# bmezaris/RetargetVid

Measured on AMD Instinct MI355X. Metric: frames/sec end-to-end saliency+crop on 640x360, higher is better.
Workload: dtype f32

## Files before the change

### retargetvid_amd/csrc/svc_tail.hip

```cpp
#include <math.h>

#include <algorithm>
#include <atomic>
#include <chrono>

#include "hdb_tree.h"
#include "svc_cvlinear.h"
#include "svc_internal.h"

#ifndef TB
#define TB 1024
#endif
#define NW16 (TB / 64)
static_assert(TB % 64 == 0 && (NW16 & (NW16 - 1)) == 0 && NW16 >= 4 && NW16 <= 16,
              "the tail kernels need 4, 8 or 16 wavefronts per workgroup");
#define RING_R 20
#define RING_R1 4
#define DEPTH_SLOT 4096
#define REACH_INF 0x1FFFFu

struct FrameWS {
    uint32_t hdr;
    uint32_t pts;
    uint32_t core;
    uint32_t mst;
    uint32_t ea, eb;
    uint32_t labels;
    uint32_t reach;
    uint32_t srt;
    uint32_t sp, ssz, absc, absw, sdn, evc, evs, dparent;
    uint32_t cup, ctp, cleft, cright, cbirthw, cminw, csize, cdn, csplit, cspa, cspb, cacc, csel, crep, cweight;
    uint32_t total;
};

static FrameWS make_layout(int cap, int mc) {
    FrameWS L;
    uint32_t o = 0;
    auto take = [&](size_t bytes) { uint32_t r = o; o += (uint32_t)((bytes + 63) / 64 * 64); return r; };
    L.hdr = take(128);
    L.pts = take(4u * cap); L.core = take(4u * cap);
    L.mst = take(8u * cap); L.ea = take(8u * cap); L.eb = take(8u * cap);
    L.labels = take(4u * cap); L.reach = take(4u * cap); L.srt = take(16u * cap + 128);
    L.sp = take(2u * cap); L.ssz = take(2u * cap); L.absc = take(2u * cap); L.absw = take(4u * cap);
    L.sdn = take(4u * cap); L.evc = take(2u * cap); L.evs = take(2u * cap);
    L.dparent = take(8u * cap);
    L.cup = take(2u * mc); L.ctp = take(4u * mc); L.cleft = take(4u * mc); L.cright = take(4u * mc);
    L.cbirthw = take(4u * mc); L.cminw = take(4u * mc); L.csize = take(4u * mc);
    L.cdn = take(4u * mc); L.csplit = take(4u * mc); L.cspa = take(4u * mc); L.cspb = take(4u * mc);
    L.cacc = take(8u * mc); L.csel = take(1u * mc);
    L.crep = take(4u * mc); L.cweight = take(4u * mc);
    L.total = o;
    return L;
}

struct TailArgs {
    uint8_t *maps;
    uint8_t *ws;
    size_t ws_stride;
    int slot0;
    const uint16_t *order;
    int n, h, w;
    FDiv dW;
    int mcs, min_samples, select_sum, op_close, clust_filt;
    int prim_pt;
    const uint32_t *ring;
    const int32_t *ring_delta;
    int n_ring, n_ring1;
    const uint16_t *ring_cnt;
    int prim_lvl;
    double *xy;
    int32_t *stats;
    FrameWS L;
};

__device__ __forceinline__ unsigned long long wave_min_u64(unsigned long long v) {
#pragma unroll
    for (int o = 32; o > 0; o >>= 1) {
        unsigned long long t = __shfl_xor(v, o);
        v = t < v ? t : v;
    }
    return v;
}
template <int CTRL, int ROW_MASK>
__device__ __forceinline__ uint32_t dpp_add_u32(uint32_t v) {
    return v + (uint32_t)__builtin_amdgcn_update_dpp(0, (int)v, CTRL, ROW_MASK, 0xF, false);
}
__device__ __forceinline__ uint32_t wave_incl_scan_u32(uint32_t v) {
    v = dpp_add_u32<0x111, 0xF>(v);
    v = dpp_add_u32<0x112, 0xF>(v);
    v = dpp_add_u32<0x114, 0xF>(v);
    v = dpp_add_u32<0x118, 0xF>(v);
    v = dpp_add_u32<0x142, 0xA>(v);
    v = dpp_add_u32<0x143, 0xC>(v);
    return v;
}

__device__ __forceinline__ int wave_sum_i32(int v) {
    return __builtin_amdgcn_readlane((int)wave_incl_scan_u32((uint32_t)v), 63);
}

template <typename T>
__device__ __forceinline__ T *carve(uint8_t *&p, size_t count) {
    T *r = (T *)p;
    p += (count * sizeof(T) + 15) / 16 * 16;
    return r;
}

__device__ __forceinline__ int block_excl_scan(int v, int *lds16, int *tot) {
    const int lane = threadIdx.x & 63, wave = threadIdx.x >> 6;
    const int inc = (int)wave_incl_scan_u32((uint32_t)v);
    if (lane == 63) lds16[wave] = inc;
    __syncthreads();
    int base = 0, total = 0;
#pragma unroll
    for (int i = 0; i < NW16; ++i) {
        int c = lds16[i];
        if (i < wave) base += c;
        total += c;
    }
    __syncthreads();
    *tot = total;
    return base + inc - v;
}

__global__ __launch_bounds__(256) void k_threshold(uint8_t *maps, size_t n, int t) {
    size_t i16 = ((size_t)blockIdx.x * 256 + threadIdx.x) * 16;
    if (i16 >= n) return;
    if (i16 + 16 <= n && (((uintptr_t)(maps + i16)) & 15) == 0) {
        uint4 v = *(uint4 *)(maps + i16);
        uint32_t *p = (uint32_t *)&v;
#pragma unroll
        for (int j = 0; j < 4; ++j) {
            uint32_t x = p[j], r = 0;
#pragma unroll
            for (int b = 0; b < 4; ++b) {
                uint32_t c = (x >> (8 * b)) & 255u;
                r |= ((int)c < t ? 0u : c) << (8 * b);
            }
            p[j] = r;
        }
        *(uint4 *)(maps + i16) = v;
    } else {
        for (size_t i = i16; i < n && i < i16 + 16; ++i) maps[i] = maps[i] < t ? 0 : maps[i];
    }
}

__global__ __launch_bounds__(256) void k_blend(uint8_t *maps, const uint16_t *order, int hw) {
    const int f = order[blockIdx.y];
    uint8_t *cur = maps + (size_t)f * hw;
    const uint8_t *prev = cur - hw;
    for (int i = blockIdx.x * 256 + threadIdx.x; i < hw; i += gridDim.x * 256)
        cur[i] = (uint8_t)(((cur[i] + prev[i]) & 255) >> 1);
}

__global__ __launch_bounds__(256) void k_iou(const int4 *__restrict__ a, const int4 *__restrict__ b, size_t n,
                                             double *__restrict__ out) {
    size_t i = (size_t)blockIdx.x * 256 + threadIdx.x;
    if (i >= n) return;
    int4 A = a[i], B = b[i];
    long long xa = max(A.x, B.x), ya = max(A.y, B.y), xb = min(A.z, B.z), yb = min(A.w, B.w);
    long long inter = max(0LL, xb - xa + 1) * max(0LL, yb - ya + 1);
    long long aa = (long long)(A.z - A.x + 1) * (A.w - A.y + 1), ab = (long long)(B.z - B.x + 1) * (B.w - B.y + 1);
    out[i] = (double)inter / (double)(aa + ab - inter);
}

__global__ __launch_bounds__(256) void k_map_resize(const uint8_t *__restrict__ in, uint8_t *__restrict__ out,
                                                    const int *__restrict__ tab, const uint16_t *__restrict__ order,
                                                    int h, int w, int oh, int ow) {
    const int f = order[blockIdx.y];
    const CvLinear T(tab, oh, ow);
    const uint8_t *src = in + (size_t)f * h * w;
    uint8_t *dst = out + (size_t)f * oh * ow;
    for (int i = blockIdx.x * 256 + threadIdx.x; i < oh * ow; i += gridDim.x * 256) {
        const int oy = i / ow, ox = i - oy * ow;
        int y0, y1, b0, b1, sx, sx1, a0, a1;
        bool inner;
        T.row(oy, h, y0, y1, b0, b1);
        T.col(ox, w, sx, sx1, a0, a1, inner);
        const uint8_t *r0 = src + (size_t)y0 * w, *r1 = src + (size_t)y1 * w;
        dst[i] = CvLinear::blend(r0[sx], r0[sx1], r1[sx], r1[sx1], a0, a1, b0, b1, inner);
    }
}

__global__ __launch_bounds__(256) void k_centre_nearest(const uint8_t *__restrict__ maps, int h, int w, int sh, int sw,
                                                        int factor, double *__restrict__ xy) {
    const int f = blockIdx.x;
    const uint8_t *m = maps + (size_t)f * h * w;
    __shared__ unsigned long long red[3 * 4];
    unsigned long long cnt = 0, sr = 0, sc = 0;
    for (int i = threadIdx.x; i < sh * sw; i += 256) {
        const int r = i / sw, c = i - r * sw;
        if (m[(size_t)min(r * factor, h - 1) * w + min(c * factor, w - 1)]) { ++cnt; sr += r; sc += c; }
    }
#pragma unroll
    for (int o = 32; o > 0; o >>= 1) { cnt += __shfl_xor(cnt, o); sr += __shfl_xor(sr, o); sc += __shfl_xor(sc, o); }
    if ((threadIdx.x & 63) == 0) { red[threadIdx.x >> 6] = cnt; red[4 + (threadIdx.x >> 6)] = sr; red[8 + (threadIdx.x >> 6)] = sc; }
    __syncthreads();
    if (threadIdx.x == 0) {
        cnt = red[0] + red[1] + red[2] + red[3];
        sr = red[4] + red[5] + red[6] + red[7];
        sc = red[8] + red[9] + red[10] + red[11];
        if (cnt) {
            xy[2 * f] = (double)sc / (double)cnt * (double)factor;
            xy[2 * f + 1] = (double)sr / (double)cnt * (double)factor;
        } else {
            xy[2 * f] = xy[2 * f + 1] = __longlong_as_double(0x7FF8000000000000LL);
        }
    }
}

__global__ __launch_bounds__(256) void k_centre_argmax(const uint8_t *__restrict__ maps, int h, int w, FDiv dW, double *__restrict__ xy) {
    const int f = blockIdx.x, hw = h * w;
    const uint8_t *m = maps + (size_t)f * hw;
    __shared__ uint32_t red[4];
    uint32_t best = 0;
    for (int i = threadIdx.x; i < hw; i += 256) best = max(best, ((uint32_t)m[i] << 16) | (uint32_t)(65535 - i));
#pragma unroll
    for (int o = 32; o > 0; o >>= 1) best = max(best, (uint32_t)__shfl_xor((int)best, o));
    if ((threadIdx.x & 63) == 0) red[threadIdx.x >> 6] = best;
    __syncthreads();
    if (threadIdx.x == 0) {
        best = max(max(red[0], red[1]), max(red[2], red[3]));
        if (best >> 16) {
            uint32_t c;
            const uint32_t r = fdivmod(65535u - (best & 0xFFFFu), dW, c);
            xy[2 * f] = (double)c;
            xy[2 * f + 1] = (double)r;
        } else {
            xy[2 * f] = xy[2 * f + 1] = __longlong_as_double(0x7FF8000000000000LL);
        }
    }
}

__device__ __forceinline__ void copy_bytes(uint8_t *__restrict__ dst, const uint8_t *__restrict__ src, int n) {
    if ((((uintptr_t)src | (uintptr_t)dst) & 7) == 0) {
        const int n8 = n >> 3;
        for (int i0 = threadIdx.x; i0 < n8; i0 += 8 * TB) {
            uint2 v[8];
#pragma unroll
            for (int u = 0; u < 8; ++u) {
                const int i = i0 + u * TB;
                v[u] = i < n8 ? ((const uint2 *)src)[i] : make_uint2(0u, 0u);
            }
#pragma unroll
            for (int u = 0; u < 8; ++u) {
                const int i = i0 + u * TB;
                if (i < n8) ((uint2 *)dst)[i] = v[u];
            }
        }
        for (int i = (n8 << 3) + threadIdx.x; i < n; i += TB) dst[i] = src[i];
    } else {
        for (int i = threadIdx.x; i < n; i += TB) dst[i] = src[i];
    }
}

__device__ __forceinline__ void compact_body(const TailArgs &A) {
    const int f = A.order[blockIdx.x];
    __shared__ int lds16[NW16];
    extern __shared__ uint8_t sm_compact[];
    const int hw = A.h * A.w;
    const uint8_t *gmap = A.maps + (size_t)f * hw;
    uint8_t *ws = A.ws + (size_t)(A.slot0 + (int)blockIdx.x) * A.ws_stride;
    uint32_t *pts = (uint32_t *)(ws + A.L.pts);
    int32_t *hdr = (int32_t *)(ws + A.L.hdr);
    uint8_t *map = sm_compact;
    copy_bytes(map, gmap, hw);
    __syncthreads();
    const int per = (hw + TB - 1) / TB;
    const int lo = min(hw, (int)threadIdx.x * per), hi = min(hw, lo + per);
    int cnt = 0;
    for (int i = lo; i < hi; ++i) cnt += map[i] != 0;
    int total;
    int pos = block_excl_scan(cnt, lds16, &total);
    if (cnt) {
        uint32_t c; uint32_t r = fdivmod((uint32_t)lo, A.dW, c);
        for (int i = lo; i < hi; ++i) {
            const uint32_t v = map[i];
            if (v) pts[pos++] = r | (c << 8) | (v << 16);
            if (++c == (uint32_t)A.w) { c = 0; ++r; }
        }
    }
    if (threadIdx.x == 0) {
        hdr[0] = total;
        hdr[1] = 0;
        hdr[2] = -1;
        hdr[3] = (A.clust_filt && total > A.mcs + 1) ? 1 : 0;
        hdr[23] = 0;
        hdr[30] = 0;
    }
}
__global__ __launch_bounds__(TB) void k_compact(TailArgs A) { compact_body(A); }

template <int NI>
__device__ __forceinline__ uint32_t core_kth_regs(const uint16_t *rcl, int N, int r, int c, int k, uint32_t lo, uint32_t hi) {
    const int lane = threadIdx.x & 63;
    uint32_t d[NI];
#pragma unroll
    for (int i = 0; i < NI; ++i) {
        const int j = lane + 64 * i;
        d[i] = 0xFFFFFFFFu;
        if (j < N) {
            const uint32_t u = rcl[j];
            const int dr = (int)(u & 255) - r, dc = (int)(u >> 8) - c;
            d[i] = (uint32_t)(dr * dr + dc * dc);
        }
    }
    auto enough = [&](uint32_t t) -> bool {
        int cnt = 0;
#pragma unroll
        for (int i = 0; i < NI; ++i) cnt += d[i] <= t;
        return wave_sum_i32(cnt) >= k + 1;
    };
    for (uint32_t t = 2 * lo; t < hi; t *= 2) {
        if (enough(t)) { hi = t; break; }
        lo = t + 1;
    }
    while (lo < hi) {
        const uint32_t mid = (lo + hi) >> 1;
        if (enough(mid)) hi = mid; else lo = mid + 1;
    }
    return lo;
}

__device__ __forceinline__ void core_body(const TailArgs &A) {
    const int f = A.order[blockIdx.x];
    uint8_t *ws = A.ws + (size_t)(A.slot0 + (int)blockIdx.x) * A.ws_stride;
    const int32_t *hdr = (const int32_t *)(ws + A.L.hdr);
    if (!hdr[3]) return;
    const int N = hdr[0];
    extern __shared__ uint8_t sm_core[];
    const int hw = A.h * A.w;
    uint8_t *occ = sm_core;
    uint32_t *ring = (uint32_t *)(sm_core + (hw + 15) / 16 * 16);
    int32_t *dl1 = (int32_t *)(ring + A.n_ring);
    __shared__ int n_fb, n_fb2;
    const uint8_t *map = A.maps + (size_t)f * hw;
    const long long tc0 = wall_clock64();
    copy_bytes(occ, map, hw);
    for (int i = threadIdx.x; i < A.n_ring; i += TB) ring[i] = A.ring[i];
    for (int i = threadIdx.x; i < A.n_ring1; i += TB) dl1[i] = A.ring_delta[i];
    if (threadIdx.x == 0) { n_fb = 0; n_fb2 = 0; }
    __syncthreads();
    const uint32_t *pts = (const uint32_t *)(ws + A.L.pts);
    uint32_t *core = (uint32_t *)(ws + A.L.core);
    int32_t *fb = (int32_t *)(ws + A.L.labels);
    int32_t *fb2 = (int32_t *)(ws + A.L.reach);
    int k = A.min_samples > 0 ? A.min_samples : A.mcs;
    k = min(N - 1, k);
    if (k == 0) k = 1;
    const int h = A.h, w = A.w;
    const int nr1 = A.n_ring1;
    for (int pbase = 0; pbase < N; pbase += TB) {
        const int p = pbase + threadIdx.x;
        const bool live = p < N;
        const uint32_t v = live ? pts[p] : 0u;
        const int r = v & 255, c = (v >> 8) & 255;
        const bool interior = r >= RING_R1 && r < h - RING_R1 && c >= RING_R1 && c < w - RING_R1;
        const uint8_t *op = occ + r * w + c;
        int cnt = 0;
        uint32_t res = live ? 0xFFFFFFFFu : 0u;
        for (int i0 = 0; i0 < nr1 && __ballot(res == 0xFFFFFFFFu) != 0ull; i0 += 8) {
            bool hit[8];
            if (interior) {
#pragma unroll
                for (int j = 0; j < 8; ++j) hit[j] = (i0 + j < nr1) && op[dl1[min(i0 + j, nr1 - 1)]] != 0;
            } else {
#pragma unroll
                for (int j = 0; j < 8; ++j) {
                    const uint32_t o = ring[min(i0 + j, nr1 - 1)];
                    const int rr = r + (int)(o & 255) - 128, cc = c + (int)((o >> 8) & 255) - 128;
                    const bool in = (i0 + j < nr1) && (unsigned)rr < (unsigned)h && (unsigned)cc < (unsigned)w;
                    hit[j] = in && occ[in ? rr * w + cc : 0] != 0;
                }
            }
            int add = 0;
#pragma unroll
            for (int j = 0; j < 8; ++j) add += hit[j] ? 1 : 0;
            if (res != 0xFFFFFFFFu) continue;
// ... 1341 lines not shown
                const double tj = readlane_f64(term, j);
                for (uint32_t k = 0; k < sj; ++k) acc += tj;
            }
        }
    }
    if (cur != hdb::NONE16 && lane == 0) t.cacc[cur] = acc;
}

template <bool LDS>
__device__ __forceinline__ int cluster_phase(const TailArgs &A, uint8_t *ws, uint8_t *sm, TreeShared &S, int32_t *hdr,
                                             int N, long long t0) {
    const int tid = threadIdx.x, nthr = blockDim.x;
    const int hw = A.h * A.w;
    hdb::Edge *ea = (hdb::Edge *)(ws + A.L.ea);
    const hdb::Edge *edges = ea;
    hdb::Tree t;
    t.dparent = (uint32_t *)(ws + A.L.dparent);
    t.nclusters = 0; t.n = N;
    if (LDS) {
        uint8_t *p = sm;
        hdb::Edge *el = carve<hdb::Edge>(p, TREE_LDS_CAP);
        t.absw = carve<uint32_t>(p, TREE_LDS_CAP); t.sdn = carve<uint32_t>(p, TREE_LDS_CAP);
        t.sp = carve<uint16_t>(p, TREE_LDS_CAP); t.ssz = carve<uint16_t>(p, TREE_LDS_CAP);
        t.absc = carve<uint16_t>(p, TREE_LDS_CAP); t.evc = carve<uint16_t>(p, TREE_LDS_CAP);
        t.evs = carve<uint16_t>(p, TREE_LDS_CAP);
        t.cacc = carve<double>(p, TREE_LDS_CLUSTERS);
        t.ctp = carve<int32_t>(p, TREE_LDS_CLUSTERS); t.cleft = carve<int32_t>(p, TREE_LDS_CLUSTERS);
        t.cright = carve<int32_t>(p, TREE_LDS_CLUSTERS); t.cbirthw = carve<uint32_t>(p, TREE_LDS_CLUSTERS);
        t.cminw = carve<uint32_t>(p, TREE_LDS_CLUSTERS); t.csize = carve<uint32_t>(p, TREE_LDS_CLUSTERS);
        t.cdn = carve<uint32_t>(p, TREE_LDS_CLUSTERS); t.csplit = carve<uint32_t>(p, TREE_LDS_CLUSTERS);
        t.cspa = carve<uint32_t>(p, TREE_LDS_CLUSTERS); t.cspb = carve<uint32_t>(p, TREE_LDS_CLUSTERS);
        t.crep = carve<int32_t>(p, TREE_LDS_CLUSTERS); t.cup = carve<uint16_t>(p, TREE_LDS_CLUSTERS);
        t.csel = carve<uint8_t>(p, TREE_LDS_CLUSTERS);
        t.cap_clusters = TREE_LDS_CLUSTERS;
        for (int i = tid; i < N - 1; i += nthr) el[i] = ea[i];
        edges = el;
    } else {
        t.sp = (uint16_t *)(ws + A.L.sp); t.ssz = (uint16_t *)(ws + A.L.ssz); t.absc = (uint16_t *)(ws + A.L.absc);
        t.absw = (uint32_t *)(ws + A.L.absw); t.sdn = (uint32_t *)(ws + A.L.sdn);
        t.evc = (uint16_t *)(ws + A.L.evc); t.evs = (uint16_t *)(ws + A.L.evs);
        t.cup = (uint16_t *)(ws + A.L.cup); t.ctp = (int32_t *)(ws + A.L.ctp); t.cleft = (int32_t *)(ws + A.L.cleft);
        t.cright = (int32_t *)(ws + A.L.cright); t.cbirthw = (uint32_t *)(ws + A.L.cbirthw);
        t.cminw = (uint32_t *)(ws + A.L.cminw); t.csize = (uint32_t *)(ws + A.L.csize);
        t.cdn = (uint32_t *)(ws + A.L.cdn); t.csplit = (uint32_t *)(ws + A.L.csplit);
        t.cspa = (uint32_t *)(ws + A.L.cspa); t.cspb = (uint32_t *)(ws + A.L.cspb); t.cacc = (double *)(ws + A.L.cacc);
        t.csel = (uint8_t *)(ws + A.L.csel); t.crep = (int32_t *)(ws + A.L.crep);
        t.cap_clusters = hdb::max_clusters(hw, A.mcs);
    }
    {
        const int per = (N + nthr - 1) / nthr;
        hdb::init_points(t, min(N, tid * per), min(N, tid * per + per));
    }
    __syncthreads();
    const bool built = build_wave(t, edges, N, A.mcs);
    if (tid == 0) hdr[13] = (int)(wall_clock64() - t0);
    if (built) accumulate_wave(t, edges);
    if (tid == 0) {
        const bool ok = built;
        if (ok) S.nsel = hdb::choose(t);
        S.ok = ok;
        hdr[4] = t.nclusters;
        hdr[9] = (int)(wall_clock64() - t0);
    }
    __syncthreads();
    if (!S.ok) return -2;
    t.nclusters = hdr[4];
    const int nsel = S.nsel;
    uint32_t *cweight = (uint32_t *)(ws + A.L.cweight);
    for (int c = tid; c < t.nclusters; c += nthr) cweight[c] = 0;
    __syncthreads();
    const uint32_t *pts = (const uint32_t *)(ws + A.L.pts);
    int32_t *labels = (int32_t *)(ws + A.L.labels);
    for (int p = tid; p < N; p += nthr) {
        const int c = hdb::point_cluster(t, (uint32_t)p, nsel);
        labels[p] = c;
        if (c >= 0) {
            const uint32_t val = pts[p] >> 16;
            if (A.select_sum == 1) atomicAdd(&cweight[c], val); else atomicMax(&cweight[c], val);
        }
    }
    __threadfence_block();
    __syncthreads();
    if (tid == 0) {
        int b = -1;
        for (int c = 0; c < t.nclusters; ++c) {
            if (t.crep[c] != c) continue;
            if (b < 0 || cweight[c] > cweight[b] || (cweight[c] == cweight[b] && hdb::cluster_before(t, c, b))) b = c;
        }
        S.best = b;
        hdr[1] = nsel;
        hdr[2] = b;
        hdr[10] = (int)(wall_clock64() - t0);
    }
    __syncthreads();
    return S.best;
}

#ifndef SORT_LDS_BYTES
#define SORT_LDS_BYTES (104 * 1024)
#endif
#define SORT_NONE 0xFFFFu
#define SORT_SMALL 15

struct SortArrays {
    uint32_t *key, *scan;
    uint16_t *idx, *seg, *lpos, *rpos;
};
struct SortSegs {
    uint16_t *lo[2], *hi[2], *pi, *ls, *rs;
// ... 149 lines not shown
    }
    for (int i = tid; i < n; i += TB) {
        const int lo = a.lpos[i], hi = a.rpos[i];
        const uint32_t k = a.key[i];
        int rank = 0;
        for (int j = lo; j <= hi; ++j) {
            const uint32_t kj = a.key[j];
            rank += (kj < k || (kj == k && j < i)) ? 1 : 0;
        }
        out[lo + rank] = a.idx[i];
    }
    __syncthreads();
}

__device__ __forceinline__ void sort_carve(uint8_t *lds, uint8_t *glob, int n, SortArrays &a, SortSegs &st, int *&sh) {
    uint8_t *p = lds;
    sh = carve<int>(p, NW16 + 4);
    const int nseg = n / 17 + 2;
    for (int g = 0; g < 2; ++g) { st.lo[g] = carve<uint16_t>(p, nseg); st.hi[g] = carve<uint16_t>(p, nseg); st.dep[g] = carve<int16_t>(p, nseg); }
    st.pi = carve<uint16_t>(p, nseg); st.ls = carve<uint16_t>(p, nseg); st.rs = carve<uint16_t>(p, nseg);
    st.vp = carve<uint32_t>(p, nseg); st.K = carve<uint32_t>(p, nseg);
    uint8_t *q = ((size_t)(p - lds) + (size_t)n * 16 + 6 * 16 <= SORT_LDS_BYTES) ? p : glob;
    a.key = carve<uint32_t>(q, n); a.scan = carve<uint32_t>(q, n);
    a.idx = carve<uint16_t>(q, n); a.seg = carve<uint16_t>(q, n); a.lpos = carve<uint16_t>(q, n); a.rpos = carve<uint16_t>(q, n);
}

__device__ __forceinline__ void sort_body(const TailArgs &A) {
    uint8_t *ws = A.ws + (size_t)(A.slot0 + (int)blockIdx.x) * A.ws_stride;
    int32_t *hdr = (int32_t *)(ws + A.L.hdr);
    if (!hdr[3]) return;
    const int n = hdr[0] - 1;
    extern __shared__ uint8_t sm_sort[];
    const long long t0 = wall_clock64();
    const hdb::Edge *mst = (const hdb::Edge *)(ws + A.L.mst);
    hdb::Edge *ea = (hdb::Edge *)(ws + A.L.ea);
    SortArrays a; SortSegs st; int *sh;
    sort_carve(sm_sort, ws + A.L.srt, n, a, st, sh);
    for (int i = threadIdx.x; i < n; i += TB) a.key[i] = mst[i].w;
    uint16_t *perm = (uint16_t *)(ws + A.L.eb);
    np_argsort_block(a, st, n, perm, sh);
    for (int i = threadIdx.x; i < n; i += TB) ea[i] = mst[perm[i]];
    if (threadIdx.x == 0) hdr[8] = (int)(wall_clock64() - t0);
}
__global__ __launch_bounds__(TB) void k_sort(TailArgs A) { sort_body(A); }

__global__ __launch_bounds__(TB) void k_argsort_test(const uint32_t *keys, int n, uint16_t *out, uint8_t *scratch) {
    extern __shared__ uint8_t sm_sort[];
    SortArrays a; SortSegs st; int *sh;
    sort_carve(sm_sort, scratch, n, a, st, sh);
    for (int i = threadIdx.x; i < n; i += TB) a.key[i] = keys[i];
    np_argsort_block(a, st, n, out, sh);
}

__global__ __launch_bounds__(64) void k_tree(TailArgs A) {
    uint8_t *ws = A.ws + (size_t)(A.slot0 + (int)blockIdx.x) * A.ws_stride;
    int32_t *hdr = (int32_t *)(ws + A.L.hdr);
    if (!hdr[3] || hdr[23]) return;
    const int N = hdr[0];
    extern __shared__ uint8_t sm_tree[];
    __shared__ TreeShared S;
    const long long t0 = wall_clock64();
    const long long c0 = clock64();
    int best = -2;
    if (N <= TREE_LDS_CAP) best = cluster_phase<true>(A, ws, sm_tree, S, hdr, N, t0);
    if (best == -2) best = cluster_phase<false>(A, ws, sm_tree, S, hdr, N, t0);
    if (threadIdx.x == 0) { hdr[14] = (int)(clock64() - c0); hdr[15] = (int)(wall_clock64() - t0); }
}

#ifndef TP_CAP
#define TP_CAP 4352
#endif
#ifndef TP_CAP_BIG
#define TP_CAP_BIG 8192
#endif
#define TP_CAP_HUGE 65025
#define TP_NONE 0xFFFFu
enum { TP_SMALL = 0, TP_BIRTH = 1, TP_SPLIT = 2, TP_ABS_A = 3, TP_ABS_B = 4 };

struct TpCl {
    double *acc;
    uint32_t *birthw, *minw, *weight;
    uint16_t *tp, *left, *right, *spa, *spb, *node, *topk, *off, *len;
    int16_t *rep;
    uint8_t *sel;
};

static size_t tp_lds_bytes(int hw, int mcs, int *cap_clusters, int *cap_clusters_huge = nullptr) {
    const int cap = std::min(hw, TP_CAP), capb = std::min(hw, TP_CAP_BIG);
    auto up = [](size_t b) { return (b + 15) / 16 * 16; };
    const size_t small = up((size_t)cap * 2) * 8 + up((size_t)(cap + 256) * 2) + up((size_t)cap * 4) * 3 + up((size_t)((cap + 256) / 16 + 16) * 2) + 64;
    const size_t big = hw > TP_CAP ? up((size_t)capb * 2) * 6 + up((size_t)(capb + 256) * 2) + up((size_t)((capb + 256) / 16 + 16) * 2) + 64 : 0;
    const size_t huge = hw > TP_CAP_BIG ? up((size_t)((hw + 256) / 16 + 16) * 2) + up(((size_t)hw / 256 + 32) * 2) + up(32 * 2) + 64 : 0;
    const size_t per_edge = std::max({small, big, huge});
    int cc = hdb::max_clusters(std::min(hw, TP_CAP_HUGE), mcs);
#ifndef TP_LDS_BUDGET
#define TP_LDS_BUDGET (160 * 1024 - 4096)
#endif
    const size_t budget = TP_LDS_BUDGET;
#ifdef TP_CC_EXACT
    if (per_edge + (size_t)cc * 48 + 512 > budget) cc = std::max(8, (int)((budget > per_edge + 512 ? budget - per_edge - 512 : 0) / 48));
#else
    while (cc > 8 && per_edge + (size_t)cc * 48 + 512 > budget) cc /= 2;
#endif
    *cap_clusters = cc;
    const size_t total = per_edge + (size_t)cc * 48 + 512;
    if (cap_clusters_huge) {
        const size_t room = total > huge + 512 ? (total - huge - 512) / 48 : 0;
        *cap_clusters_huge = (int)std::min<size_t>(room, (size_t)hdb::max_clusters(std::min(hw, TP_CAP_HUGE), mcs));
    }
    return total;
}

__device__ __forceinline__ uint32_t tp_gt_mask16(const uint16_t *p, uint32_t r) {
    const uint4 a = ((const uint4 *)p)[0], b = ((const uint4 *)p)[1];
    const uint32_t v[8] = {a.x, a.y, a.z, a.w, b.x, b.y, b.z, b.w};
    uint32_t m = 0;
#pragma unroll
    for (int i = 0; i < 8; ++i) m |= ((v[i] & 0xFFFFu) > r ? 1u << (2 * i) : 0u) | ((v[i] >> 16) > r ? 2u << (2 * i) : 0u);
    return m;
}
// ... 304 lines not shown
            const uint32_t val = pts[pid] >> 16;
            if (A.select_sum == 1) atomicAdd(&C.weight[lab], val); else atomicMax(&C.weight[lab], val);
        }
    }
    __syncthreads();
    if (tid == 0) {
        auto depth = [&](uint32_t k) { int d = 0; while (par[k] != TP_NONE) { k = par[k]; ++d; } return d; };
        auto before = [&](int c1, int c2) -> bool {
            const uint32_t p1 = C.tp[c1], p2 = C.tp[c2];
            if (p1 == TP_NONE) return true;
            if (p2 == TP_NONE) return false;
            if (p1 == p2) return C.left[p1] == c1;
            uint32_t s1 = C.node[p1], s2 = C.node[p2];
            const int d1 = depth(s1), d2 = depth(s2);
            if (d1 != d2) return d1 < d2;
            uint32_t side1 = 0, side2 = 0;
            while (s1 != s2) {
                side1 = s1 > par[s1]; side2 = s2 > par[s2];
                s1 = par[s1]; s2 = par[s2];
            }
            return side1 < side2;
        };
        int b = -1;
        for (int c = 0; c < nc; ++c) {
            if (C.rep[c] != c) continue;
            if (b < 0 || C.weight[c] > C.weight[b] || (C.weight[c] == C.weight[b] && before(c, b))) b = c;
        }
        hdr[1] = nsel;
        hdr[2] = b;
        hdr[23] = 1;
        hdr[10] = (int)(wall_clock64() - t0);
        hdr[15] = hdr[10];
    }
}
#undef TP_ORDER
#undef TP_W

__device__ __forceinline__ void tree_par_body(const TailArgs &A, int cap_clusters, int cap_clusters_huge) {
    uint8_t *ws = A.ws + (size_t)(A.slot0 + (int)blockIdx.x) * A.ws_stride;
    int32_t *hdr = (int32_t *)(ws + A.L.hdr);
    if (!hdr[3]) return;
    const int N = hdr[0];
    if (N > TP_CAP_HUGE) return;
    extern __shared__ uint8_t sm_tp[];
    __shared__ int lds16[NW16];
    __shared__ int sh_nc, sh_nsel;
    if (N <= TP_CAP) tp_body<0>(A, cap_clusters, ws, hdr, N, sm_tp, lds16, sh_nc, sh_nsel);
    else if (N <= TP_CAP_BIG) tp_body<1>(A, cap_clusters, ws, hdr, N, sm_tp, lds16, sh_nc, sh_nsel);
    else tp_body<2>(A, cap_clusters_huge, ws, hdr, N, sm_tp, lds16, sh_nc, sh_nsel);
}
__global__ __launch_bounds__(TB) void k_tree_par(TailArgs A, int cap_clusters, int cap_clusters_huge) { tree_par_body(A, cap_clusters, cap_clusters_huge); }

__device__ __forceinline__ void finish_body(const TailArgs &A) {
    const int f = A.order[blockIdx.x];
    uint8_t *ws = A.ws + (size_t)(A.slot0 + (int)blockIdx.x) * A.ws_stride;
    int32_t *hdr = (int32_t *)(ws + A.L.hdr);
    if (hdr[30]) return;
    const int N = hdr[0];
    const int hw = A.h * A.w;
    uint8_t *map = A.maps + (size_t)f * hw;
    extern __shared__ uint8_t sm_fin[];
    __shared__ unsigned long long red[3 * NW16];
    __shared__ uint32_t box[4];
    const int tid = threadIdx.x;
    if (tid < 4) box[tid] = 255u;
    const bool clustered = hdr[3] != 0;
    long long t0 = 0;
    if (tid == 0) t0 = wall_clock64();
    const int best = clustered ? hdr[2] : -1;
    uint8_t *m0 = sm_fin;
    uint8_t *m1 = sm_fin + (hw + 15) / 16 * 16;
    copy_bytes(m0, map, hw);
    __syncthreads();
    int wr0 = 0, wc0 = 0, wh = A.h, ww = A.w;
    if (best >= 0) {
        const uint32_t *pts = (const uint32_t *)(ws + A.L.pts);
        const int32_t *labels = (const int32_t *)(ws + A.L.labels);
        uint32_t rmin = 255, cmin = 255, rmaxc = 255, cmaxc = 255;
        for (int p = tid; p < N; p += TB) {
            const uint32_t v = pts[p], r = v & 255, c = (v >> 8) & 255;
            if (labels[p] != best) m0[r * A.w + c] = 0;
            else { rmin = min(rmin, r); cmin = min(cmin, c); rmaxc = min(rmaxc, 255u - r); cmaxc = min(cmaxc, 255u - c); }
        }
        const uint32_t a = wave_min_u32(rmin), b = wave_min_u32(cmin), c_ = wave_min_u32(rmaxc), d = wave_min_u32(cmaxc);
        if ((tid & 63) == 0) { atomicMin(&box[0], a); atomicMin(&box[1], b); atomicMin(&box[2], c_); atomicMin(&box[3], d); }
        __syncthreads();
        if (box[0] <= 255u - box[2]) {
            wr0 = max(0, (int)box[0] - 4); wc0 = max(0, (int)box[1] - 4);
            wh = min(A.h, (int)(255u - box[2]) + 5) - wr0; ww = min(A.w, (int)(255u - box[3]) + 5) - wc0;
        }
        if (A.op_close) {
            close_pass<true, true>(m0, m1, A.w, wr0, wc0, wh, ww);
            __syncthreads();
            close_pass<true, false>(m1, m0, A.w, wr0, wc0, wh, ww);
            __syncthreads();
            close_pass<false, true>(m0, m1, A.w, wr0, wc0, wh, ww);
            __syncthreads();
            close_pass<false, false>(m1, m0, A.w, wr0, wc0, wh, ww);
            __syncthreads();
        }
        copy_bytes(map, m0, hw);
    }
    __syncthreads();
    unsigned long long cnt = 0, sr = 0, sc = 0;
    for (int i = tid; i < wh * ww; i += TB) {
        const int r = wr0 + i / ww, c = wc0 + i % ww;
        if (m0[r * A.w + c]) { ++cnt; sr += (uint32_t)r; sc += (uint32_t)c; }
    }
    cnt = (unsigned long long)(uint32_t)wave_sum_i32((int)cnt);
    sr = (unsigned long long)(uint32_t)wave_sum_i32((int)sr);
    sc = (unsigned long long)(uint32_t)wave_sum_i32((int)sc);
    if ((tid & 63) == 0) { red[tid >> 6] = cnt; red[NW16 + (tid >> 6)] = sr; red[2 * NW16 + (tid >> 6)] = sc; }
    __syncthreads();
    if (tid == 0) {
        cnt = sr = sc = 0;
        for (int i = 0; i < NW16; ++i) { cnt += red[i]; sr += red[NW16 + i]; sc += red[2 * NW16 + i]; }
        if (cnt) {
            A.xy[2 * f] = (double)sc / (double)cnt;
            A.xy[2 * f + 1] = (double)sr / (double)cnt;
        } else {
            A.xy[2 * f] = A.xy[2 * f + 1] = __longlong_as_double(0x7FF8000000000000LL);
        }
        if (A.stats) {
            A.stats[4 * f] = N;
            A.stats[4 * f + 1] = clustered ? hdr[1] : 0;
            A.stats[4 * f + 2] = clustered ? hdr[2] : -1;
            A.stats[4 * f + 3] = (int)cnt;
        }
        hdr[11] = (int)(wall_clock64() - t0);
    }
}
__global__ __launch_bounds__(TB) void k_finish(TailArgs A) { finish_body(A); }

__global__ __launch_bounds__(TB) void k_tail_front(TailArgs A) {
    compact_body(A);
    __syncthreads();
    core_body(A);
    __syncthreads();
    prim_lvl_body(A);
}

__global__ __launch_bounds__(TB) void k_tail_back(TailArgs A, int cap_clusters, int cap_clusters_huge) {
    int32_t *hdr = (int32_t *)(A.ws + (size_t)(A.slot0 + (int)blockIdx.x) * A.ws_stride + A.L.hdr);
    sort_body(A);
    __syncthreads();
    tree_par_body(A, cap_clusters, cap_clusters_huge);
    __syncthreads();
    if (hdr[3] && !hdr[23]) return;
    finish_body(A);
    __syncthreads();
    if (threadIdx.x == 0) hdr[30] = 1;
}

extern "C" int svc_threshold_u8(SvcHandle *h, uint8_t *maps, size_t n_bytes, int t, void *stream) {
    if (!h || (n_bytes > 0 && !maps)) { svc_set_error("svc_threshold_u8: invalid argument"); return SVC_E_INVALID; }
    if (n_bytes == 0) return SVC_OK;
    SVC_HIP(hipSetDevice(h->device));
    ProfScope ps(h, SVC_K_THRESHOLD, (hipStream_t)stream);
    k_threshold<<<(unsigned)((n_bytes + 4095) / 4096), 256, 0, (hipStream_t)stream>>>(maps, n_bytes, t);
    SVC_CHECK_LAUNCH();
    return SVC_OK;
}

extern "C" int svc_iou_i32(const int32_t *a, const int32_t *b, size_t n, double *out, void *stream) {
    if (!a || !b || !out) { svc_set_error("svc_iou_i32: invalid argument"); return SVC_E_INVALID; }
    if (n == 0) return SVC_OK;
    k_iou<<<(unsigned)((n + 255) / 256), 256, 0, (hipStream_t)stream>>>((const int4 *)a, (const int4 *)b, n, out);
    SVC_CHECK_LAUNCH();
    return SVC_OK;
}

static int upload_map_tab(DevBuf &buf, int h, int w, int oh, int ow, double sy, double sx) {
    const std::vector<int> tab = cv_linear_tab(h, w, oh, ow, sy, sx);
    int rc = buf.ensure(tab.size() * 4);
    if (rc) return rc;
    SVC_HIP(hipMemcpy(buf.p, tab.data(), tab.size() * 4, hipMemcpyHostToDevice));
    return SVC_OK;
}

#define RC_TAIL(x) do { int rc_ = (x); if (rc_) return rc_; } while (0)

static int ensure_ring(SvcHandle *h) {
    if (h->tail_n_offsets) return SVC_OK;
    std::vector<uint32_t> v;
    for (int dr = -RING_R; dr <= RING_R; ++dr)
        for (int dc = -RING_R; dc <= RING_R; ++dc) {
            int d2 = dr * dr + dc * dc;
            if (d2 == 0 || d2 > RING_R * RING_R) continue;
            v.push_back((uint32_t)(dr + 128) | ((uint32_t)(dc + 128) << 8) | ((uint32_t)d2 << 16));
        }
    std::stable_sort(v.begin(), v.end(), [](uint32_t x, uint32_t y) { return (x >> 16) < (y >> 16); });
    int rc = h->tail_offsets.ensure(v.size() * 4);
    if (rc) return rc;
    SVC_HIP(hipMemcpy(h->tail_offsets.p, v.data(), v.size() * 4, hipMemcpyHostToDevice));
    h->tail_offsets_host = v;
    h->tail_n_offsets = (int)v.size();
    h->tail_n_offsets1 = 0;
    for (uint32_t x : v) h->tail_n_offsets1 += (int)((x >> 16) <= RING_R1 * RING_R1);
    std::vector<uint16_t> cnt(RING_R * RING_R + 1, 0);
    for (uint32_t x : v) ++cnt[x >> 16];
    for (size_t m = 1; m < cnt.size(); ++m) cnt[m] = (uint16_t)(cnt[m] + cnt[m - 1]);
// ... 90 lines not shown
    if (params->resize_factor < 1 || params->resize_factor > 16) { svc_set_error("svc_cluster_center: resize_factor must be an integer in 1..16"); return SVC_E_INVALID; }
    if (n == 0) return SVC_OK;
    SVC_HIP(hipSetDevice(h->device));
    hipStream_t s = (hipStream_t)stream;
    int rc = ensure_ring(h);
    if (rc) return rc;
    const int full_h = height, full_w = width;
    const int rs_h = (int)lrint((double)full_h * (1.0 / params->resize_factor));
    const int rs_w = (int)lrint((double)full_w * (1.0 / params->resize_factor));
    if (params->resize_factor > 1 && (params->clust_filt || params->com_km) && (rs_h < 1 || rs_w < 1)) {
        svc_set_error("svc_cluster_center: map %dx%d too small for resize_factor %d", full_h, full_w, params->resize_factor);
        return SVC_E_INVALID;
    }
    const int factor = params->clust_filt ? params->resize_factor : 1;
    uint8_t *full_maps = maps;
    const int *rs_down = nullptr, *rs_up = nullptr;
    if (factor > 1) {
        height = rs_h;
        width = rs_w;
        auto key = std::make_tuple(full_h, full_w, factor);
        auto it = h->rs_tabs.find(key);
        if (it == h->rs_tabs.end()) {
            std::pair<DevBuf, DevBuf> t;
            if ((rc = upload_map_tab(t.first, full_h, full_w, height, width, (double)factor, (double)factor))) return rc;
            if ((rc = upload_map_tab(t.second, height, width, full_h, full_w, (double)height / full_h, (double)width / full_w))) return rc;
            it = h->rs_tabs.emplace(key, t).first;
        }
        rs_down = (const int *)it->second.first.p;
        rs_up = (const int *)it->second.second.p;
        if ((rc = h->rs_maps.ensure((size_t)n * height * width))) return rc;
        maps = (uint8_t *)h->rs_maps.p;
    }
    const int cap = height * width;
    const int mc = hdb::max_clusters(cap, params->hdbscan_min);
    FrameWS L = make_layout(cap, mc);
    const int HELD = 255;
    std::vector<uint8_t> depth;
    std::vector<uint16_t> blend0;
    int maxd = 0;
    if ((rc = plan_rounds(blend_flags_host, n, depth, blend0, maxd))) return rc;
    if (n > DEPTH_SLOT) { svc_set_error("svc_cluster_center: more than %d maps per call", DEPTH_SLOT); return SVC_E_INVALID; }
    std::vector<uint16_t> order(2 * (size_t)n, 0);
    std::vector<int> round_start(maxd + 2, 0);
    for (int i = 0; i < n; ++i) if (depth[i] != HELD) ++round_start[depth[i] + 1];
    for (int r = 0; r <= maxd; ++r) round_start[r + 1] += round_start[r];
    {
        std::vector<int> fill(round_start.begin(), round_start.end() - 1);
        for (int i = 0; i < n; ++i) if (depth[i] != HELD) order[fill[depth[i]]++] = (uint16_t)i;
    }
    for (size_t i = 0; i < blend0.size(); ++i) order[n + i] = blend0[i];
    const size_t lists_bytes = 8 * 4 * (size_t)DEPTH_SLOT;
    const int n_proc = round_start[maxd + 1];
    if ((rc = h->tail_ws.ensure(lists_bytes + (size_t)L.total * std::max<size_t>(32, ((size_t)n_proc + 31) / 32 * 32)))) return rc;
    if (!h->depth_pinned) SVC_HIP(hipHostMalloc((void **)&h->depth_pinned, 8 * 4 * (size_t)DEPTH_SLOT, hipHostMallocDefault));
    const int slot = h->depth_slot++ & 7;
    if (h->depth_ev[slot]) SVC_HIP(hipEventSynchronize(h->depth_ev[slot]));
    else SVC_HIP(hipEventCreateWithFlags(&h->depth_ev[slot], hipEventDisableTiming));
    uint16_t *order_dev = (uint16_t *)((uint8_t *)h->tail_ws.p + (size_t)slot * 4 * DEPTH_SLOT);
    memcpy(h->depth_pinned + (size_t)slot * 4 * DEPTH_SLOT, order.data(), (size_t)n * 4);
    SVC_HIP(hipMemcpyAsync(order_dev, h->depth_pinned + (size_t)slot * 4 * DEPTH_SLOT, (size_t)n * 4, hipMemcpyHostToDevice, s));
    SVC_HIP(hipEventRecord(h->depth_ev[slot], s));
    h->tail_frames = n; h->tail_h = height; h->tail_w = width; h->tail_frame_stride = L.total;
    h->tail_slot_of.assign((size_t)n, -1);
    for (int i = 0; i < n_proc; ++i) h->tail_slot_of[order[i]] = i;
    TailArgs A;
    A.maps = maps; A.ws = (uint8_t *)h->tail_ws.p + lists_bytes; A.ws_stride = L.total; A.order = order_dev; A.slot0 = 0;
    A.n = n; A.h = height; A.w = width; A.dW = make_fdiv(width);
    A.mcs = params->hdbscan_min; A.min_samples = params->hdbscan_min_samples; A.select_sum = params->select_sum;
    A.op_close = params->op_close; A.clust_filt = params->clust_filt;
    A.prim_pt = h->prim_pt;
    const int32_t *ring_delta = nullptr;
    RC_TAIL(ensure_ring_delta(h, width, &ring_delta));
    A.ring = (const uint32_t *)h->tail_offsets.p; A.n_ring = h->tail_n_offsets; A.n_ring1 = h->tail_n_offsets1;
    A.ring_delta = ring_delta;
    A.ring_cnt = (const uint16_t *)h->tail_ring_cnt.p; A.prim_lvl = h->prim_lvl;
    A.xy = xy; A.stats = stats; A.L = L;
    const int hw = height * width;
    const size_t lds_core = (size_t)(hw + 15) / 16 * 16 + (size_t)h->tail_n_offsets * 4 + (size_t)h->tail_n_offsets1 * 4;
    const size_t lds_prim = 2 * NW16 * 16 + (size_t)hw * 2;
    const size_t lds_fin = 2 * ((size_t)(hw + 15) / 16 * 16);
    if (h->lds_attr_done.insert((const void *)k_core).second) {
        SVC_HIP(hipFuncSetAttribute((const void *)k_core, hipFuncAttributeMaxDynamicSharedMemorySize, 160 * 1024 - 1024));
        SVC_HIP(hipFuncSetAttribute((const void *)k_prim_pt<2>, hipFuncAttributeMaxDynamicSharedMemorySize, 160 * 1024 - 1024));
        SVC_HIP(hipFuncSetAttribute((const void *)k_prim_pt<4>, hipFuncAttributeMaxDynamicSharedMemorySize, 160 * 1024 - 1024));
        SVC_HIP(hipFuncSetAttribute((const void *)k_prim_pt<8>, hipFuncAttributeMaxDynamicSharedMemorySize, 160 * 1024 - 1024));
        SVC_HIP(hipFuncSetAttribute((const void *)k_prim_big, hipFuncAttributeMaxDynamicSharedMemorySize, 160 * 1024 - 1024));
        SVC_HIP(hipFuncSetAttribute((const void *)k_prim_lvl, hipFuncAttributeMaxDynamicSharedMemorySize, 160 * 1024 - 256));
        SVC_HIP(hipFuncSetAttribute((const void *)k_prim_lvl_big, hipFuncAttributeMaxDynamicSharedMemorySize, 160 * 1024 - 1024));
        SVC_HIP(hipFuncSetAttribute((const void *)k_finish, hipFuncAttributeMaxDynamicSharedMemorySize, 160 * 1024 - 8 * 1024));
        SVC_HIP(hipFuncSetAttribute((const void *)k_tree, hipFuncAttributeMaxDynamicSharedMemorySize, 160 * 1024 - 8 * 1024));
        SVC_HIP(hipFuncSetAttribute((const void *)k_tree_par, hipFuncAttributeMaxDynamicSharedMemorySize, 160 * 1024 - 1024));
        SVC_HIP(hipFuncSetAttribute((const void *)k_tail_front, hipFuncAttributeMaxDynamicSharedMemorySize, 160 * 1024 - 256));
        SVC_HIP(hipFuncSetAttribute((const void *)k_tail_back, hipFuncAttributeMaxDynamicSharedMemorySize, 160 * 1024 - 1024));
        SVC_HIP(hipFuncSetAttribute((const void *)k_sort, hipFuncAttributeMaxDynamicSharedMemorySize, SORT_LDS_BYTES));
    }
    for (int r = 0; r <= maxd; ++r) {
        const int m = round_start[r + 1] - round_start[r];
        const uint16_t *ord = order_dev + round_start[r];
        A.order = ord; A.slot0 = round_start[r];
        if (r == 0 && !blend0.empty()) {
            k_blend<<<dim3(8, (unsigned)blend0.size()), 256, 0, s>>>(full_maps, order_dev + n, full_h * full_w);
            SVC_CHECK_LAUNCH();
        }
        if (m == 0) continue;
        if (r > 0) {
            k_blend<<<dim3(8, m), 256, 0, s>>>(full_maps, ord, full_h * full_w);
            SVC_CHECK_LAUNCH();
        }
        if (factor > 1) {
            k_map_resize<<<dim3(8, m), 256, 0, s>>>(full_maps, maps, rs_down, ord, full_h, full_w, height, width);
            SVC_CHECK_LAUNCH();
        }
        int cap_cl = 0, cap_cl_huge = 0;
        const size_t lds_tp = tp_lds_bytes(hw, params->hdbscan_min, &cap_cl, &cap_cl_huge);
        const bool tree_fallback = !h->tree_par || hw > TP_CAP_HUGE || hdb::max_clusters(std::min(hw, TP_CAP_BIG), params->hdbscan_min) > cap_cl ||
                                   (hw > TP_CAP_BIG && hdb::max_clusters(std::min(hw, TP_CAP_HUGE), params->hdbscan_min) > cap_cl_huge);
        if (params->clust_filt && h->tail_merge && h->prim_lvl && h->tree_par) {
            const size_t lds_front = std::max({(size_t)(hw + 15) / 16 * 16, lds_core, lvl_lds_bytes(height, width, h->tail_n_offsets)});
            const size_t lds_back = std::max({(size_t)SORT_LDS_BYTES, lds_tp, lds_fin});
            {
                ProfScope ps(h, SVC_K_PRIM, s);
                k_tail_front<<<m, TB, lds_front, s>>>(A);
                SVC_CHECK_LAUNCH();
                if (hw > LVL_CAP) { k_prim_lvl_big<<<m, TB, lvl_big_lds_bytes(height, width, h->tail_n_offsets), s>>>(A); SVC_CHECK_LAUNCH(); }
            }
            ProfScope ps(h, SVC_K_FINISH, s);
            k_tail_back<<<m, TB, lds_back, s>>>(A, cap_cl, cap_cl_huge);
            SVC_CHECK_LAUNCH();
            if (tree_fallback) {
                k_tree<<<m, 64, FIN_LDS_BYTES, s>>>(A);
                SVC_CHECK_LAUNCH();
                k_finish<<<m, TB, lds_fin, s>>>(A);
                SVC_CHECK_LAUNCH();
            }
        } else {
        {
            ProfScope ps(h, SVC_K_COMPACT, s);
            k_compact<<<m, TB, (size_t)(hw + 15) / 16 * 16, s>>>(A);
            SVC_CHECK_LAUNCH();
        }
        if (params->clust_filt) {
            {
                ProfScope ps(h, SVC_K_CORE, s);
                k_core<<<m, TB, lds_core, s>>>(A);
                SVC_CHECK_LAUNCH();
            }
            ProfScope ps(h, SVC_K_PRIM, s);
            const int n_min = h->prim_lvl ? LVL_CAP : 0;
            if (h->prim_lvl) {
                k_prim_lvl<<<m, TB, lvl_lds_bytes(height, width, h->tail_n_offsets), s>>>(A);
                SVC_CHECK_LAUNCH();
            } else {
                if (h->prim_pt <= 2) { k_prim_pt<2><<<m, TB, lds_prim, s>>>(A, n_min); SVC_CHECK_LAUNCH(); }
                if (h->prim_pt <= 4 && (hw > 2 * TB || h->prim_pt > 2)) { k_prim_pt<4><<<m, TB, lds_prim, s>>>(A, n_min); SVC_CHECK_LAUNCH(); }
                if (hw > 4 * TB || h->prim_pt > 4) { k_prim_pt<8><<<m, TB, lds_prim, s>>>(A, n_min); SVC_CHECK_LAUNCH(); }
            }
            if (hw > LVL_CAP && h->prim_lvl) { k_prim_lvl_big<<<m, TB, lvl_big_lds_bytes(height, width, h->tail_n_offsets), s>>>(A); SVC_CHECK_LAUNCH(); }
            else if (hw > 8 * TB) { k_prim_big<<<m, TB, lds_prim, s>>>(A, n_min); SVC_CHECK_LAUNCH(); }
        }
        {
            ProfScope ps(h, SVC_K_FINISH, s);
            if (params->clust_filt) {
                k_sort<<<m, TB, SORT_LDS_BYTES, s>>>(A);
                SVC_CHECK_LAUNCH();
                if (h->tree_par) {
                    k_tree_par<<<m, TB, lds_tp, s>>>(A, cap_cl, cap_cl_huge);
                    SVC_CHECK_LAUNCH();
                }
                if (tree_fallback) {
                    k_tree<<<m, 64, FIN_LDS_BYTES, s>>>(A);
                    SVC_CHECK_LAUNCH();
                }
            }
            k_finish<<<m, TB, lds_fin, s>>>(A);
            SVC_CHECK_LAUNCH();
        }
        }
        if (factor > 1) {
            k_map_resize<<<dim3(16, m), 256, 0, s>>>(maps, full_maps, rs_up, ord, height, width, full_h, full_w);
            SVC_CHECK_LAUNCH();
        }
    }
    if (!params->com_km) {
        k_centre_argmax<<<n, 256, 0, s>>>(full_maps, full_h, full_w, make_fdiv(full_w), xy);
        SVC_CHECK_LAUNCH();
    } else if (params->resize_factor > 1) {
        k_centre_nearest<<<n, 256, 0, s>>>(full_maps, full_h, full_w, rs_h, rs_w, params->resize_factor, xy);
// ... 56 lines not shown
```

Baseline: 25980.

## Fold blend, order upload and fallback tree kernels into fused tail kernels

Moves the temporal map blend into the compact stage of the fused front kernel when no resize is needed, blending while copying the map into LDS. The per-round frame order is passed inline in kernel arguments when small, so the pinned-buffer upload, event sync and H2D copy are skipped. The big-level prim pass and the serial tree plus finish fallback are also folded into the front and back kernels, which cuts kernel launches per round. In exchange the kernel arguments get larger, LDS sizing becomes the max of more stages, and the serial tree fallback now runs on one wave inside a full workgroup.

New measurement: 25960 (median of 2 runs). No clear change (-0.1%).

```diff
diff --git a/retargetvid_amd/csrc/svc_tail.hip b/retargetvid_amd/csrc/svc_tail.hip
--- a/retargetvid_amd/csrc/svc_tail.hip
+++ b/retargetvid_amd/csrc/svc_tail.hip
@@ -18,6 +18,8 @@
 #define RING_R1 4
 #define DEPTH_SLOT 4096
 #define REACH_INF 0x1FFFFu
+#define TAIL_ORDER_INL 128
+#define TAIL_BLEND_FIRST 0x8000u
 
 struct FrameWS {
     uint32_t hdr;
@@ -71,7 +73,13 @@
     double *xy;
     int32_t *stats;
     FrameWS L;
+    uint16_t order_inl[TAIL_ORDER_INL];
 };
+
+__device__ __forceinline__ uint32_t tail_entry(const TailArgs &A) {
+    return A.order ? A.order[blockIdx.x] : A.order_inl[A.slot0 + (int)blockIdx.x];
+}
+__device__ __forceinline__ int tail_map(const TailArgs &A) { return (int)(tail_entry(A) & (TAIL_BLEND_FIRST - 1u)); }
 
 __device__ __forceinline__ unsigned long long wave_min_u64(unsigned long long v) {
 #pragma unroll
@@ -145,12 +153,20 @@
     }
 }
 
+__device__ __forceinline__ uint32_t blend_u8(uint32_t cur, uint32_t prev) { return ((cur + prev) & 255u) >> 1; }
+__device__ __forceinline__ uint32_t blend_u8x4(uint32_t cur, uint32_t prev) {
+    uint32_t r = 0;
+#pragma unroll
+    for (int b = 0; b < 32; b += 8) r |= blend_u8((cur >> b) & 255u, (prev >> b) & 255u) << b;
+    return r;
+}
+
 __global__ __launch_bounds__(256) void k_blend(uint8_t *maps, const uint16_t *order, int hw) {
     const int f = order[blockIdx.y];
     uint8_t *cur = maps + (size_t)f * hw;
     const uint8_t *prev = cur - hw;
     for (int i = blockIdx.x * 256 + threadIdx.x; i < hw; i += gridDim.x * 256)
-        cur[i] = (uint8_t)(((cur[i] + prev[i]) & 255) >> 1);
+        cur[i] = (uint8_t)blend_u8(cur[i], prev[i]);
 }
 
 __global__ __launch_bounds__(256) void k_iou(const int4 *__restrict__ a, const int4 *__restrict__ b, size_t n,
@@ -254,17 +270,43 @@
     }
 }
 
+__device__ __forceinline__ void copy_blend_bytes(uint8_t *__restrict__ dst, uint8_t *cur, const uint8_t *prev, int n) {
+    if ((((uintptr_t)cur | (uintptr_t)prev | (uintptr_t)dst) & 7) == 0) {
+        const int n8 = n >> 3;
+        for (int i0 = threadIdx.x; i0 < n8; i0 += 4 * TB) {
+            uint2 c[4], p[4];
+#pragma unroll
+            for (int u = 0; u < 4; ++u) {
+                const int i = i0 + u * TB;
+                c[u] = i < n8 ? ((const uint2 *)cur)[i] : make_uint2(0u, 0u);
+                p[u] = i < n8 ? ((const uint2 *)prev)[i] : make_uint2(0u, 0u);
+            }
+#pragma unroll
+            for (int u = 0; u < 4; ++u) {
+                const int i = i0 + u * TB;
+                const uint2 v = make_uint2(blend_u8x4(c[u].x, p[u].x), blend_u8x4(c[u].y, p[u].y));
+                if (i < n8) { ((uint2 *)dst)[i] = v; ((uint2 *)cur)[i] = v; }
+            }
+        }
+        for (int i = (n8 << 3) + threadIdx.x; i < n; i += TB) dst[i] = cur[i] = (uint8_t)blend_u8(cur[i], prev[i]);
+    } else {
+        for (int i = threadIdx.x; i < n; i += TB) dst[i] = cur[i] = (uint8_t)blend_u8(cur[i], prev[i]);
+    }
+}
+
 __device__ __forceinline__ void compact_body(const TailArgs &A) {
-    const int f = A.order[blockIdx.x];
+    const uint32_t ent = tail_entry(A);
+    const int f = (int)(ent & (TAIL_BLEND_FIRST - 1u));
     __shared__ int lds16[NW16];
     extern __shared__ uint8_t sm_compact[];
     const int hw = A.h * A.w;
-    const uint8_t *gmap = A.maps + (size_t)f * hw;
+    uint8_t *gmap = A.maps + (size_t)f * hw;
     uint8_t *ws = A.ws + (size_t)(A.slot0 + (int)blockIdx.x) * A.ws_stride;
     uint32_t *pts = (uint32_t *)(ws + A.L.pts);
     int32_t *hdr = (int32_t *)(ws + A.L.hdr);
     uint8_t *map = sm_compact;
-    copy_bytes(map, gmap, hw);
+    if (ent & TAIL_BLEND_FIRST) copy_blend_bytes(map, gmap, gmap - hw, hw);
+    else copy_bytes(map, gmap, hw);
     __syncthreads();
     const int per = (hw + TB - 1) / TB;
     const int lo = min(hw, (int)threadIdx.x * per), hi = min(hw, lo + per);
@@ -323,7 +365,7 @@
 }
 
 __device__ __forceinline__ void core_body(const TailArgs &A) {
-    const int f = A.order[blockIdx.x];
+    const int f = tail_map(A);
     uint8_t *ws = A.ws + (size_t)(A.slot0 + (int)blockIdx.x) * A.ws_stride;
     const int32_t *hdr = (const int32_t *)(ws + A.L.hdr);
     if (!hdr[3]) return;
@@ -1771,9 +1813,12 @@
         hdb::init_points(t, min(N, tid * per), min(N, tid * per + per));
     }
     __syncthreads();
-    const bool built = build_wave(t, edges, N, A.mcs);
-    if (tid == 0) hdr[13] = (int)(wall_clock64() - t0);
-    if (built) accumulate_wave(t, edges);
+    bool built = false;
+    if (tid < 64) {
+        built = build_wave(t, edges, N, A.mcs);
+        if (tid == 0) hdr[13] = (int)(wall_clock64() - t0);
+        if (built) accumulate_wave(t, edges);
+    }
     if (tid == 0) {
         const bool ok = built;
         if (ok) S.nsel = hdb::choose(t);
@@ -2029,7 +2074,7 @@
     np_argsort_block(a, st, n, out, sh);
 }
 
-__global__ __launch_bounds__(64) void k_tree(TailArgs A) {
+__device__ __forceinline__ void tree_serial_body(const TailArgs &A) {
     uint8_t *ws = A.ws + (size_t)(A.slot0 + (int)blockIdx.x) * A.ws_stride;
     int32_t *hdr = (int32_t *)(ws + A.L.hdr);
     if (!hdr[3] || hdr[23]) return;
@@ -2043,6 +2088,7 @@
     if (best == -2) best = cluster_phase<false>(A, ws, sm_tree, S, hdr, N, t0);
     if (threadIdx.x == 0) { hdr[14] = (int)(clock64() - c0); hdr[15] = (int)(wall_clock64() - t0); }
 }
+__global__ __launch_bounds__(64) void k_tree(TailArgs A) { tree_serial_body(A); }
 
 #ifndef TP_CAP
 #define TP_CAP 4352
@@ -2453,7 +2499,7 @@
 __global__ __launch_bounds__(TB) void k_tree_par(TailArgs A, int cap_clusters, int cap_clusters_huge) { tree_par_body(A, cap_clusters, cap_clusters_huge); }
 
 __device__ __forceinline__ void finish_body(const TailArgs &A) {
-    const int f = A.order[blockIdx.x];
+    const int f = tail_map(A);
     uint8_t *ws = A.ws + (size_t)(A.slot0 + (int)blockIdx.x) * A.ws_stride;
     int32_t *hdr = (int32_t *)(ws + A.L.hdr);
     if (hdr[30]) return;
@@ -2539,15 +2585,21 @@
     core_body(A);
     __syncthreads();
     prim_lvl_body(A);
-}
-
-__global__ __launch_bounds__(TB) void k_tail_back(TailArgs A, int cap_clusters, int cap_clusters_huge) {
+    __syncthreads();
+    prim_lvl_big_body(A);
+}
+
+__global__ __launch_bounds__(TB) void k_tail_back(TailArgs A, int cap_clusters, int cap_clusters_huge, int serial) {
     int32_t *hdr = (int32_t *)(A.ws + (size_t)(A.slot0 + (int)blockIdx.x) * A.ws_stride + A.L.hdr);
     sort_body(A);
     __syncthreads();
     tree_par_body(A, cap_clusters, cap_clusters_huge);
     __syncthreads();
-    if (hdr[3] && !hdr[23]) return;
+    if (hdr[3] && !hdr[23]) {
+        if (!serial) return;
+        tree_serial_body(A);
+        __syncthreads();
+    }
     finish_body(A);
     __syncthreads();
     if (threadIdx.x == 0) hdr[30] = 1;
@@ -2744,18 +2796,33 @@
     const size_t lists_bytes = 8 * 4 * (size_t)DEPTH_SLOT;
     const int n_proc = round_start[maxd + 1];
     if ((rc = h->tail_ws.ensure(lists_bytes + (size_t)L.total * std::max<size_t>(32, ((size_t)n_proc + 31) / 32 * 32)))) return rc;
-    if (!h->depth_pinned) SVC_HIP(hipHostMalloc((void **)&h->depth_pinned, 8 * 4 * (size_t)DEPTH_SLOT, hipHostMallocDefault));
-    const int slot = h->depth_slot++ & 7;
-    if (h->depth_ev[slot]) SVC_HIP(hipEventSynchronize(h->depth_ev[slot]));
-    else SVC_HIP(hipEventCreateWithFlags(&h->depth_ev[slot], hipEventDisableTiming));
-    uint16_t *order_dev = (uint16_t *)((uint8_t *)h->tail_ws.p + (size_t)slot * 4 * DEPTH_SLOT);
-    memcpy(h->depth_pinned + (size_t)slot * 4 * DEPTH_SLOT, order.data(), (size_t)n * 4);
-    SVC_HIP(hipMemcpyAsync(order_dev, h->depth_pinned + (size_t)slot * 4 * DEPTH_SLOT, (size_t)n * 4, hipMemcpyHostToDevice, s));
-    SVC_HIP(hipEventRecord(h->depth_ev[slot], s));
     h->tail_frames = n; h->tail_h = height; h->tail_w = width; h->tail_frame_stride = L.total;
     h->tail_slot_of.assign((size_t)n, -1);
     for (int i = 0; i < n_proc; ++i) h->tail_slot_of[order[i]] = i;
+    const bool fused = params->clust_filt && h->tail_merge && h->prim_lvl && h->tree_par;
+    const bool blend_in_front = fused && factor == 1;
+    const bool order_inline = blend_in_front && n_proc <= TAIL_ORDER_INL;
+    if (blend_in_front) {
+        for (int i = round_start[1]; i < n_proc; ++i) order[i] |= (uint16_t)TAIL_BLEND_FIRST;
+        std::vector<uint8_t> first(n, 0);
+        for (uint16_t i : blend0) first[i] = 1;
+        for (int i = 0; i < round_start[1]; ++i) if (first[order[i]]) order[i] |= (uint16_t)TAIL_BLEND_FIRST;
+    }
     TailArgs A;
+    uint16_t *order_dev = nullptr;
+    memset(A.order_inl, 0, sizeof A.order_inl);
+    if (order_inline) {
+        memcpy(A.order_inl, order.data(), (size_t)n_proc * 2);
+    } else {
+        if (!h->depth_pinned) SVC_HIP(hipHostMalloc((void **)&h->depth_pinned, 8 * 4 * (size_t)DEPTH_SLOT, hipHostMallocDefault));
+        const int slot = h->depth_slot++ & 7;
+        if (h->depth_ev[slot]) SVC_HIP(hipEventSynchronize(h->depth_ev[slot]));
+        else SVC_HIP(hipEventCreateWithFlags(&h->depth_ev[slot], hipEventDisableTiming));
+        order_dev = (uint16_t *)((uint8_t *)h->tail_ws.p + (size_t)slot * 4 * DEPTH_SLOT);
+        memcpy(h->depth_pinned + (size_t)slot * 4 * DEPTH_SLOT, order.data(), (size_t)n * 4);
+        SVC_HIP(hipMemcpyAsync(order_dev, h->depth_pinned + (size_t)slot * 4 * DEPTH_SLOT, (size_t)n * 4, hipMemcpyHostToDevice, s));
+        SVC_HIP(hipEventRecord(h->depth_ev[slot], s));
+    }
     A.maps = maps; A.ws = (uint8_t *)h->tail_ws.p + lists_bytes; A.ws_stride = L.total; A.order = order_dev; A.slot0 = 0;
     A.n = n; A.h = height; A.w = width; A.dW = make_fdiv(width);
     A.mcs = params->hdbscan_min; A.min_samples = params->hdbscan_min_samples; A.select_sum = params->select_sum;
@@ -2788,14 +2855,14 @@
     }
     for (int r = 0; r <= maxd; ++r) {
         const int m = round_start[r + 1] - round_start[r];
-        const uint16_t *ord = order_dev + round_start[r];
+        const uint16_t *ord = order_inline ? nullptr : order_dev + round_start[r];
         A.order = ord; A.slot0 = round_start[r];
-        if (r == 0 && !blend0.empty()) {
+        if (r == 0 && !blend0.empty() && !blend_in_front) {
             k_blend<<<dim3(8, (unsigned)blend0.size()), 256, 0, s>>>(full_maps, order_dev + n, full_h * full_w);
             SVC_CHECK_LAUNCH();
         }
         if (m == 0) continue;
-        if (r > 0) {
+        if (r > 0 && !blend_in_front) {
             k_blend<<<dim3(8, m), 256, 0, s>>>(full_maps, ord, full_h * full_w);
             SVC_CHECK_LAUNCH();
         }
@@ -2807,24 +2874,18 @@
         const size_t lds_tp = tp_lds_bytes(hw, params->hdbscan_min, &cap_cl, &cap_cl_huge);
         const bool tree_fallback = !h->tree_par || hw > TP_CAP_HUGE || hdb::max_clusters(std::min(hw, TP_CAP_BIG), params->hdbscan_min) > cap_cl ||
                                    (hw > TP_CAP_BIG && hdb::max_clusters(std::min(hw, TP_CAP_HUGE), params->hdbscan_min) > cap_cl_huge);
-        if (params->clust_filt && h->tail_merge && h->prim_lvl && h->tree_par) {
-            const size_t lds_front = std::max({(size_t)(hw + 15) / 16 * 16, lds_core, lvl_lds_bytes(height, width, h->tail_n_offsets)});
-            const size_t lds_back = std::max({(size_t)SORT_LDS_BYTES, lds_tp, lds_fin});
+        if (fused) {
+            const size_t lds_front = std::max({(size_t)(hw + 15) / 16 * 16, lds_core, lvl_lds_bytes(height, width, h->tail_n_offsets),
+                                               hw > LVL_CAP ? lvl_big_lds_bytes(height, width, h->tail_n_offsets) : (size_t)0});
+            const size_t lds_back = std::max({(size_t)SORT_LDS_BYTES, lds_tp, lds_fin, tree_fallback ? (size_t)FIN_LDS_BYTES : (size_t)0});
             {
                 ProfScope ps(h, SVC_K_PRIM, s);
                 k_tail_front<<<m, TB, lds_front, s>>>(A);
                 SVC_CHECK_LAUNCH();
-                if (hw > LVL_CAP) { k_prim_lvl_big<<<m, TB, lvl_big_lds_bytes(height, width, h->tail_n_offsets), s>>>(A); SVC_CHECK_LAUNCH(); }
             }
             ProfScope ps(h, SVC_K_FINISH, s);
-            k_tail_back<<<m, TB, lds_back, s>>>(A, cap_cl, cap_cl_huge);
+            k_tail_back<<<m, TB, lds_back, s>>>(A, cap_cl, cap_cl_huge, tree_fallback ? 1 : 0);
             SVC_CHECK_LAUNCH();
-            if (tree_fallback) {
-                k_tree<<<m, 64, FIN_LDS_BYTES, s>>>(A);
-                SVC_CHECK_LAUNCH();
-                k_finish<<<m, TB, lds_fin, s>>>(A);
-                SVC_CHECK_LAUNCH();
-            }
         } else {
         {
             ProfScope ps(h, SVC_K_COMPACT, s);
```
